# simonsobs/Pixell.jl

Measured on AMD Instinct MI355X. Metric: Mpix/s CAR bilinear reproject (Float64) + % HBM roofline, 1/2/4/8 MI355X, higher is better.
Workload: dtype f64

## Files before the change

### pixell.jl_amd/csrc/pxl_kernels.hip

```cpp
#include <hip/hip_runtime.h>

#include <algorithm>
#include <mutex>
#include <vector>
#include <cmath>
#include <cstdarg>
#include <cstdio>
#include <cstring>
#include <new>
#include <type_traits>

#include "pxl_device.h"

using namespace pxl;

static thread_local char g_err[512] = "";

static int fail(int code, const char* fmt, ...) {
    va_list ap;
    va_start(ap, fmt);
    vsnprintf(g_err, sizeof(g_err), fmt, ap);
    va_end(ap);
    return code;
}
#define HIP_TRY(expr)                                                                         \
    do {                                                                                      \
        hipError_t e_ = (expr);                                                               \
        if (e_ != hipSuccess) return fail(PXL_EHIP, "%s: %s", #expr, hipGetErrorString(e_));  \
    } while (0)

static int check_launch(const char* what) {
    hipError_t e = hipGetLastError();
    if (e != hipSuccess) return fail(PXL_EHIP, "launch of %s failed: %s", what, hipGetErrorString(e));
    return PXL_OK;
}

static bool wcs_ok(const pxl_car_wcs* w) {
    if (!w) return false;
    for (int k = 0; k < 2; ++k)
        if (!std::isfinite(w->cdelt[k]) || !std::isfinite(w->crpix[k]) || !std::isfinite(w->crval[k]) ||
            w->cdelt[k] == 0.0)
            return false;
    return std::isfinite(w->unit) && w->unit != 0.0;
}

static inline unsigned stream_grid(int64_t work_items, int block) {
    int64_t nb = (work_items + block - 1) / block;
    if (nb < 1) nb = 1;
    if (nb > (1LL << 20)) nb = 1LL << 20;
    return (unsigned)nb;
}

static int env_int(const char* name, int dflt) {
    const char* v = getenv(name);
    return (v && *v) ? atoi(v) : dflt;
}

#include "pxl_elementwise.h"
#include "pxl_unwrap.h"
#include "pxl_maps.h"
#include "pxl_fastmath.h"
#include "pxl_tan.h"
#include "pxl_reproject.h"
#include "pxl_reproject_dma.h"
#include "pxl_sample.h"
#include "pxl_misc.h"
#include "pxl_rccl.h"
#include "pxl_spread.h"
#include "pxl_distance.h"
#include "pxl_spline.h"

static constexpr size_t PXL_RING_BYTES = 17 * 1024;
static constexpr int64_t PXL_MIN_TILES = 8192;

struct pxl_reproject_plan {
    pxl_car_wcs win, wout;
    int64_t nx, ny, nc, src_row0, src_nrows;
    int64_t nxo, nyo, dst_row0, dst_nrows;
    int periodic;
    int device;
    int32_t* xi0; double* xfx; int32_t* yj0; double* yfy;
    void* table_mem;
    int32_t* h_yj0;
    int variant;
    int pairs;
    int pairs_dma;
    int seg_dma;
    int pairs_dma32;
    int seg_dma32;
    bool dma32_ok;
    int dypos;
    int rh;
    int rh32;
    int seg;
    int dxpos;
    int ns, pf;
    int nt;
    double* zero_page;
    bool staged_ok;
    bool vec_load;
    bool tables_built;
    hipStream_t comm_stream;
    hipEvent_t ev_ready, ev_halo;
    int64_t cov_have_lo, cov_have_hi, cov_lo, cov_hi;
};

struct UnwindWs {
    char* base;
    int8_t* c; int32_t* rloc; int32_t* bsum; int32_t* boff;
    int32_t* flag;
    unsigned long long* firstnan;
    int2* wsum; double2* wprev;
    UwLink* links; unsigned int* ticket; int64_t nlinks;
    int64_t nb, nw;
    int U;
    bool multipass;
};

static const int64_t kUnwindBlockFallbackMax = 1LL << 22;


static std::mutex g_pool_mu;
static hipMemPool_t g_pools[64] = {};
static hipMemPool_t unwind_pool() {
    std::mutex& mu = g_pool_mu;
    hipMemPool_t* pools = g_pools;
    int dev = 0;
    if (hipGetDevice(&dev) != hipSuccess || dev < 0 || dev >= 64) return nullptr;
    std::lock_guard<std::mutex> lock(mu);
    if (!pools[dev]) {
        hipMemPoolProps props = {};
        props.allocType = hipMemAllocationTypePinned;
        props.location.type = hipMemLocationTypeDevice;
        props.location.id = dev;
        hipMemPool_t p = nullptr;
        if (hipMemPoolCreate(&p, &props) != hipSuccess) { (void)hipGetLastError(); return nullptr; }
        uint64_t keep = ~0ull;
        (void)hipMemPoolSetAttribute(p, hipMemPoolAttrReleaseThreshold, &keep);
        pools[dev] = p;
    }
    return pools[dev];
}

static int unwind_ws_alloc(int64_t n, int nrow, hipStream_t st, UnwindWs* w) {
    w->nb = (n + PXL_SCAN_BLOCK - 1) / PXL_SCAN_BLOCK;
    int64_t U = n / (64 * 4096);
    U = U < 4 ? 4 : (U > 32 ? 32 : U);
    U &= ~(int64_t)(PXL_UW_G - 1);
    w->U = (int)U;
    w->nw = (n + 64 * U - 1) / (64 * U);
    if (w->nb > 0x7fffffffLL || w->nw > 0x7fffffffLL || n > 0x7fffffffLL) return fail(PXL_EINVAL, "unwind: batch too long (2^31 points)");
    auto up = [](size_t b) { return (b + 255) & ~(size_t)255; };
    w->multipass = n > kUnwindBlockFallbackMax;
    const size_t bytes_c = w->multipass ? up((size_t)nrow * n) : 0, bytes_r = w->multipass ? up((size_t)4 * nrow * n) : 0,
                 bytes_b = w->multipass ? up((size_t)4 * nrow * w->nb) : 0;
    const size_t bytes_ws = up((size_t)w->nw * sizeof(int2)), bytes_wp = up((size_t)w->nw * sizeof(double2));
    w->nlinks = (n + PXL_UW1_CHUNK - 1) / PXL_UW1_CHUNK;
    const size_t bytes_ln = up((size_t)w->nlinks * sizeof(UwLink) + 16);
    const size_t total = bytes_c + bytes_r + 2 * bytes_b + bytes_ws + bytes_wp + bytes_ln + 256;
    w->base = nullptr;
    hipMemPool_t pool = unwind_pool();
    if (pool) HIP_TRY(hipMallocFromPoolAsync((void**)&w->base, total, pool, st));
    else HIP_TRY(hipMallocAsync((void**)&w->base, total, st));
    char* p = w->base;
    w->c = (int8_t*)p; p += bytes_c;
    w->rloc = (int32_t*)p; p += bytes_r;
    w->bsum = (int32_t*)p; p += bytes_b;
    w->boff = (int32_t*)p; p += bytes_b;
    w->wsum = (int2*)p; p += bytes_ws;
    w->wprev = (double2*)p; p += bytes_wp;
    w->links = (UwLink*)p; w->ticket = (unsigned int*)(p + (size_t)w->nlinks * sizeof(UwLink)); p += bytes_ln;
    w->flag = (int32_t*)p;
    w->firstnan = (unsigned long long*)(p + 16);
    if (hipMemsetAsync(w->flag, 0, 32, st) != hipSuccess) {
        (void)hipFreeAsync(w->base, st);
        return fail(PXL_EHIP, "unwind: hipMemsetAsync failed");
    }
    return PXL_OK;
}

static int unwind_ws_free(UnwindWs* w, hipStream_t st, int rc) {
    hipError_t e = hipFreeAsync(w->base, st);
    if (e != hipSuccess && rc == PXL_OK) rc = fail(PXL_EHIP, "unwind: hipFreeAsync: %s", hipGetErrorString(e));
    return rc;
}

template <class SRC>
static int unwind_fused(const SRC& src, typename SRC::raw_t* out, int64_t n, bool inplace, UnwindWs& w, hipStream_t st) {
    const dim3 grid((unsigned)w.nw), block(64);
    int32_t* fastflag = w.flag + 2;
    hipLaunchKernelGGL((k_unwind_sums<SRC>), grid, block, 0, st, src, n, w.U, w.wsum, w.wprev, w.firstnan);
    hipLaunchKernelGGL(k_scan_wsums, dim3(1), dim3(1024), 0, st, w.nw, w.wsum);
    if (inplace) {
        hipLaunchKernelGGL((k_unwind_apply<SRC, false>), grid, block, 0, st, src, out, n, w.U, (const int2*)w.wsum,
                           (const double2*)w.wprev, (const unsigned long long*)w.firstnan, fastflag, (const int32_t*)nullptr);
        hipLaunchKernelGGL((k_unwind_apply<SRC, true>), grid, block, 0, st, src, out, n, w.U, (const int2*)w.wsum,
                           (const double2*)w.wprev, (const unsigned long long*)w.firstnan, fastflag, (const int32_t*)fastflag);
    } else {
        hipLaunchKernelGGL((k_unwind_apply<SRC, true>), grid, block, 0, st, src, out, n, w.U, (const int2*)w.wsum,
                           (const double2*)w.wprev, (const unsigned long long*)w.firstnan, fastflag, (const int32_t*)nullptr);
    }
    return check_launch("k_unwind fused");
}

template <class SRC>
static int unwind_onepass(const SRC& src, typename SRC::raw_t* out, int64_t n, UnwindWs& w, hipStream_t st) {
    if (w.nlinks > 0x7fffffffLL) return fail(PXL_EINVAL, "unwind: batch too long");
    hipError_t e = hipMemsetAsync(w.links, 0, (size_t)w.nlinks * sizeof(UwLink) + 16, st);
    if (e != hipSuccess) return fail(PXL_EHIP, "unwind: hipMemsetAsync: %s", hipGetErrorString(e));
    const int64_t nwg = (n + PXL_UW1_CHUNK - 1) / PXL_UW1_CHUNK;
    hipLaunchKernelGGL((k_unwind_onepass<SRC, PXL_UW1_U, PXL_UW1_UL>), dim3((unsigned)nwg), dim3(64 * PXL_UW1_WAVES), 0, st, src, out, n, w.links, w.ticket, w.flag + 2);
    return check_launch("k_unwind_onepass");
}

static int unwind_multipass(int64_t n, int nrow, double* sky, double period, double ref, UnwindWs& w, const int32_t* gate,
                            hipStream_t st) {
    int rc = PXL_OK;
    const unsigned cap = gate ? 2048u : 0xffffffffu;
    const unsigned g = std::min(stream_grid(n, 256), cap);
    const int64_t nb = w.nb;
    hipLaunchKernelGGL(k_unwrap_incr, dim3(g), dim3(256), 0, st, n, nrow, (const double*)sky, period, w.c, gate);
    for (int pass = 0; pass < 2 && rc == PXL_OK; ++pass) {
        const int32_t* pg = pass == 0 ? gate : w.flag;
        hipLaunchKernelGGL((k_scan_local<int8_t>), dim3(std::min((unsigned)nb, cap), nrow), dim3(256), 0, st, n, (const int8_t*)w.c, w.rloc, w.bsum, nb, pg);
        hipLaunchKernelGGL(k_scan_bsums, dim3(nrow), dim3(1024), 0, st, nb, (const int32_t*)w.bsum, w.boff, pg);
        hipLaunchKernelGGL(k_unwrap_verify, dim3(g), dim3(256), 0, st, n, nrow, (const double*)sky, period, w.c,
                           (const int32_t*)w.rloc, (const int32_t*)w.boff, nb, w.flag + pass, pg);
        rc = check_launch("k_unwrap scan/verify");
    }
    if (rc == PXL_OK) {
        hipLaunchKernelGGL(k_unwrap_apply, dim3(g), dim3(256), 0, st, n, nrow, sky, period, ref, (const int32_t*)w.rloc,
                           (const int32_t*)w.boff, nb, (const int32_t*)w.flag, gate);
        hipLaunchKernelGGL(k_unwind_rows, dim3(nrow), dim3(64), 0, st, n, nrow, sky, period, ref, 1, (const int32_t*)w.flag);
        rc = check_launch("k_unwrap_apply");
    }
    return rc;
}


extern "C" {

int pxl_version(void) { return PXL_VERSION; }

size_t pxl_last_error(char* buf, size_t n) {
    size_t len = strlen(g_err);
    if (buf && n) {
        size_t m = len < n - 1 ? len : n - 1;
        memcpy(buf, g_err, m);
        buf[m] = 0;
    }
// ... 269 lines not shown
    auto up256 = [](size_t b) { return (b + 255) & ~(size_t)255; };
    const size_t npix = (size_t)nx * (size_t)ny;
    const size_t b_csa = up256((size_t)nx * 16), b_csd = up256((size_t)ny * 16), b_best = up256(npix * 4), b_chain = npix * 8;
    hipStream_t st = (hipStream_t)stream;
    char* ws = nullptr;
    hipMemPool_t pool = unwind_pool();
    if (pool) HIP_TRY(hipMallocFromPoolAsync((void**)&ws, b_csa + b_csd + b_best + b_chain, pool, st));
    else HIP_TRY(hipMallocAsync((void**)&ws, b_csa + b_csd + b_best + b_chain, st));
    double2* csa = (double2*)ws;
    double2* csd = (double2*)(ws + b_csa);
    int32_t* best = (int32_t*)(ws + b_csa + b_csd);
    long long* chain = (long long*)(ws + b_csa + b_csd + b_best);
    hipLaunchKernelGGL(k_sdt_tables, dim3(stream_grid(nx + ny, 256)), dim3(256), 0, st, c, nx, ny, csa, csd);
    const size_t lds = (size_t)((nx + 63) / 64) * 16;
    hipLaunchKernelGGL(k_sdt_rows, dim3((unsigned)ny), dim3(PXL_SDT_ROW_THREADS), lds, st, m, nx, (const double2*)csa, best);
    hipLaunchKernelGGL(k_sdt_columns, dim3((unsigned)((nx + 63) / 64)), dim3(64), 0, st, (const int32_t*)best, nx, ny, up ? 1 : 0,
                       (const double2*)csa, (const double2*)csd, chain, dist);
    int rc = check_launch("k_sdt_rows / k_sdt_columns");
    hipError_t fe = hipFreeAsync(ws, st);
    if (fe != hipSuccess && rc == PXL_OK) rc = fail(PXL_EHIP, "distance_transform: hipFreeAsync: %s", hipGetErrorString(fe));
    return rc;
}

int pxl_sky2pix_tan_f64(const pxl_car_wcs* wcs, int64_t n, const double* ra, const double* dec, double* ipix,
                        double* jpix, void* stream) {
    if (!wcs_ok(wcs)) return fail(PXL_EINVAL, "sky2pix_tan: invalid WCS");
    if (n < 0 || (n > 0 && (!ipix || !jpix || !ra || !dec))) return fail(PXL_EINVAL, "sky2pix_tan: null buffer or negative n");
    if (n == 0) return PXL_OK;
    const bool vec = ((((uintptr_t)ra | (uintptr_t)dec | (uintptr_t)ipix | (uintptr_t)jpix) & 15) == 0);
    const dim3 grid(stream_grid((n + 1) / 2, 256));
    if (vec) hipLaunchKernelGGL((k_tan_points<true, false>), grid, dim3(256), 0, (hipStream_t)stream, tan_setup(*wcs), n, ra, dec, ipix, jpix);
    else     hipLaunchKernelGGL((k_tan_points<false, false>), grid, dim3(256), 0, (hipStream_t)stream, tan_setup(*wcs), n, ra, dec, ipix, jpix);
    return check_launch("k_tan_points (sky2pix)");
}

int pxl_pix2sky_tan_f64(const pxl_car_wcs* wcs, int64_t n, const double* ipix, const double* jpix, double* ra,
                        double* dec, void* stream) {
    if (!wcs_ok(wcs)) return fail(PXL_EINVAL, "pix2sky_tan: invalid WCS");
    if (n < 0 || (n > 0 && (!ipix || !jpix || !ra || !dec))) return fail(PXL_EINVAL, "pix2sky_tan: null buffer or negative n");
    if (n == 0) return PXL_OK;
    const bool vec = ((((uintptr_t)ra | (uintptr_t)dec | (uintptr_t)ipix | (uintptr_t)jpix) & 15) == 0);
    const dim3 grid(stream_grid((n + 1) / 2, 256));
    if (vec) hipLaunchKernelGGL((k_tan_points<true, true>), grid, dim3(256), 0, (hipStream_t)stream, tan_setup(*wcs), n, ipix, jpix, ra, dec);
    else     hipLaunchKernelGGL((k_tan_points<false, true>), grid, dim3(256), 0, (hipStream_t)stream, tan_setup(*wcs), n, ipix, jpix, ra, dec);
    return check_launch("k_tan_points (pix2sky)");
}

int pxl_posmap_tan_f64(const pxl_car_wcs* wcs, const int64_t shape[2], int64_t row0, int64_t nrows, double* ra,
                       double* dec, void* stream) {
    if (!wcs_ok(wcs)) return fail(PXL_EINVAL, "posmap_tan: invalid WCS");
    int rc = check_rows("posmap_tan", shape, row0, nrows);
    if (rc) return rc;
    if (nrows == 0) return PXL_OK;
    if (!ra || !dec) return fail(PXL_EINVAL, "posmap_tan: null output");
    const int64_t nchunk = (shape[0] + 511) / 512;
    const int64_t nrb = (nrows + PXL_TAN_ROWS - 1) / PXL_TAN_ROWS;
    if (nchunk * nrb > 0x7fffffffLL) return fail(PXL_EINVAL, "posmap_tan: map too large for one launch");
    const bool vec = (shape[0] % 2 == 0) && ((((uintptr_t)ra | (uintptr_t)dec) & 15) == 0);
    const TanParams tp0 = tan_setup(*wcs);
    const bool grid_pays = fabs(tp0.uos) * PXL_TG_W <= 0.04 && fabs(tp0.cd0) >= 0.3;
    if (grid_pays && shape[0] >= PXL_TG_W && nrows >= 8) {
        const int64_t ntx = (shape[0] + PXL_TG_W - 1) / PXL_TG_W, nty = (nrows + PXL_TG_ROWS - 1) / PXL_TG_ROWS;
        int fronts = 8;
        if (nty < 4 * fronts) fronts = 1;
        const int64_t per = (nty + fronts - 1) / fronts, nbx = (ntx + 3) / 4;
        const int64_t nblk = per * fronts * nbx;
        if (nblk <= 0x7fffffffLL) {
            if (vec) hipLaunchKernelGGL((k_posmap_tan_grid<true>), dim3((unsigned)nblk), dim3(256), 0, (hipStream_t)stream, tp0, shape[0], row0, nrows, ntx, per, fronts, ra, dec);
            else     hipLaunchKernelGGL((k_posmap_tan_grid<false>), dim3((unsigned)nblk), dim3(256), 0, (hipStream_t)stream, tp0, shape[0], row0, nrows, ntx, per, fronts, ra, dec);
            return check_launch("k_posmap_tan_grid");
        }
    }
    const dim3 grid((unsigned)(nchunk * nrb));
    if (vec) hipLaunchKernelGGL((k_posmap_tan<true>), grid, dim3(256), 0, (hipStream_t)stream, tan_setup(*wcs), shape[0], row0, nrows, nchunk, ra, dec);
    else     hipLaunchKernelGGL((k_posmap_tan<false>), grid, dim3(256), 0, (hipStream_t)stream, tan_setup(*wcs), shape[0], row0, nrows, nchunk, ra, dec);
    return check_launch("k_posmap_tan");
}


int pxl_reproject_plan_create(const pxl_car_wcs* wcs_in, const int64_t shape_in[3], int64_t src_row0,
                              int64_t src_nrows, const pxl_car_wcs* wcs_out, const int64_t shape_out[2],
                              int64_t dst_row0, int64_t dst_nrows, pxl_reproject_plan** out) {
    if (!out) return fail(PXL_EINVAL, "plan_create: null plan pointer");
    *out = nullptr;
    if (!wcs_ok(wcs_in) || !wcs_ok(wcs_out)) return fail(PXL_EINVAL, "plan_create: invalid WCS");
    if (!shape_in || !shape_out) return fail(PXL_EINVAL, "plan_create: null shape");
    if (shape_in[0] < 1 || shape_in[1] < 1 || shape_in[2] < 1 || shape_out[0] < 1 || shape_out[1] < 1)
        return fail(PXL_EINVAL, "plan_create: shapes must be positive");
    if (shape_in[0] > 400000000 || shape_in[1] > 1000000000 || shape_out[0] > 1000000000 || shape_out[1] > 1000000000)
        return fail(PXL_EINVAL, "plan_create: axis too long (source RA axis <= 4e8, others <= 1e9 pixels)");
    if (src_row0 < 0 || src_nrows < 0 || src_row0 + src_nrows > shape_in[1])
        return fail(PXL_EINVAL, "plan_create: source window outside the map");
    if (dst_row0 < 0 || dst_nrows < 0 || dst_row0 + dst_nrows > shape_out[1])
        return fail(PXL_EINVAL, "plan_create: destination window outside the map");

    pxl_reproject_plan* pl = new (std::nothrow) pxl_reproject_plan();
    if (!pl) return fail(PXL_ENOMEM, "plan_create: host allocation failed");
    pl->cov_lo = 0; pl->cov_hi = -1;
    pl->win = *wcs_in; pl->wout = *wcs_out;
    pl->nx = shape_in[0]; pl->ny = shape_in[1]; pl->nc = shape_in[2];
    pl->src_row0 = src_row0; pl->src_nrows = src_nrows;
    pl->nxo = shape_out[0]; pl->nyo = shape_out[1];
    pl->dst_row0 = dst_row0; pl->dst_nrows = dst_nrows;
    pl->periodic = fabs((double)pl->nx * fabs(wcs_in->cdelt[0] * wcs_in->unit) - PXL_TWOPI_D) < 1e-8;
    pl->tables_built = false;

    hipError_t e = hipGetDevice(&pl->device);
    if (e != hipSuccess) { delete pl; return fail(PXL_ENODEV, "hipGetDevice: %s", hipGetErrorString(e)); }

    size_t nxo = (size_t)pl->nxo, nyo = (size_t)pl->nyo;
    size_t off_xfx = 0;
    size_t off_yfy = off_xfx + ((nxo * 8 + 15) & ~(size_t)15);
    size_t off_xi0 = off_yfy + ((nyo * 8 + 15) & ~(size_t)15);
    size_t off_yj0 = off_xi0 + ((nxo * 4 + 15) & ~(size_t)15);
    size_t off_zero = off_yj0 + ((nyo * 4 + 15) & ~(size_t)15);
    size_t total = off_zero + 64;
    e = hipMalloc(&pl->table_mem, total);
    if (e != hipSuccess) { delete pl; return fail(PXL_ENOMEM, "plan_create: hipMalloc(%zu): %s", total, hipGetErrorString(e)); }
    char* base = (char*)pl->table_mem;
    e = hipMemset(base + off_zero, 0, 64);
    if (e != hipSuccess) { (void)hipFree(pl->table_mem); delete pl; return fail(PXL_EHIP, "plan_create: hipMemset: %s", hipGetErrorString(e)); }
    pl->zero_page = (double*)(base + off_zero);
    pl->xfx = (double*)(base + off_xfx); pl->yfy = (double*)(base + off_yfy);
    pl->xi0 = (int32_t*)(base + off_xi0); pl->yj0 = (int32_t*)(base + off_yj0);

    pl->h_yj0 = new (std::nothrow) int32_t[nyo];
    if (!pl->h_yj0) { (void)hipFree(pl->table_mem); delete pl; return fail(PXL_ENOMEM, "plan_create: host allocation failed"); }
    CarAffine co = car_affine(pl->wout);
    Sky2Pix si = sky2pix_setup(pl->win, pl->nx, pl->ny, 1, PXL_FORM_DIV);
    for (int64_t j = 0; j < pl->nyo; ++j) {
        double fr;
        split_cell(s2p_y(si, p2s_dec(co, (double)(j + 1))), &pl->h_yj0[j], &fr);
    }

    double sx = fabs((pl->wout.cdelt[0] * pl->wout.unit) / (pl->win.cdelt[0] * pl->win.unit));
    pl->dxpos = ((pl->wout.cdelt[0] * pl->wout.unit) / (pl->win.cdelt[0] * pl->win.unit)) > 0 ? 1 : 0;
    pl->dypos = ((pl->wout.cdelt[1] * pl->wout.unit) / (pl->win.cdelt[1] * pl->win.unit)) > 0 ? 1 : 0;
    double sy = fabs((pl->wout.cdelt[1] * pl->wout.unit) / (pl->win.cdelt[1] * pl->win.unit));
    pl->rh = env_int("PXL_REPROJECT_RH", sy >= 1.5 ? 4 : (sy > 0.3 ? 16 : 8));
    if (pl->rh < 1) pl->rh = 1;
    if (pl->rh > 64) pl->rh = 64;
    pl->rh32 = env_int("PXL_REPROJECT_RH", 32);
    if (pl->rh32 < 1) pl->rh32 = 1;
    if (pl->rh32 > 64) pl->rh32 = 64;
    pl->ns = env_int("PXL_REPROJECT_NS", (double)pl->nx * (double)pl->ny * (double)pl->nc * 8.0 <= 128.0 * 1048576.0 ? 4 : 8);
    if (pl->ns < 4) pl->ns = 4;
    while (pl->ns & (pl->ns - 1)) pl->ns &= pl->ns - 1;
    if (pl->ns > 64) pl->ns = 64;
    {
        int want_pf = (int)ceil((pl->ns - 2) / (sy > 0.125 ? sy : 0.125));
        pl->pf = env_int("PXL_REPROJECT_PF", want_pf < 3 ? 3 : want_pf);
    }
    pl->nt = env_int("PXL_REPROJECT_NT", 1);
    if (pl->pf < 0) pl->pf = 0;
    const int max_seg = PXL_MAXCH * 128;
    auto seg_for = [&](int pairs) -> int64_t {
        double span = ceil((double)(128 * pairs) * sx) + 5.0;
        int64_t s = (int64_t)span;
        return (s + 1) & ~(int64_t)1;
    };
    int want = env_int("PXL_REPROJECT_PAIRS", sx <= 0.55 ? 4 : 2);
    if (want != 1 && want != 2 && want != 4) want = 2;
    pl->pairs_dma = want;
    while (pl->pairs_dma > 1 && seg_for(pl->pairs_dma) > max_seg) pl->pairs_dma >>= 1;
    pl->seg_dma = (int)std::min<int64_t>(seg_for(pl->pairs_dma), max_seg);
    pl->pairs = want > 2 ? 2 : want;
    if (seg_for(pl->pairs) > max_seg && pl->pairs == 2) pl->pairs = 1;
    int64_t seg = seg_for(pl->pairs);
    auto stageable = [&](int64_t sg) { return (sg <= max_seg) && !(pl->periodic && sg > pl->nx) && sy <= 3.0; };
    pl->staged_ok = stageable(seg) && stageable(seg_for(pl->pairs_dma));
    pl->seg = (int)(seg <= max_seg ? seg : max_seg);
    {
        const int max_seg32 = PXL_MAXCH * 256;
        auto seg_for32 = [&](int pairs) -> int64_t {
            double span = ceil((double)(256 * pairs) * sx) + 8.0;
            return ((int64_t)span + 3) & ~(int64_t)3;
        };
        pl->pairs_dma32 = env_int("PXL_REPROJECT_PAIRS", sx < 0.75 ? 1 : 2);
        if (pl->pairs_dma32 != 1 && pl->pairs_dma32 != 2 && pl->pairs_dma32 != 4) pl->pairs_dma32 = 2;
        while (pl->pairs_dma32 > 1 && seg_for32(pl->pairs_dma32) > max_seg32) pl->pairs_dma32 >>= 1;
        int64_t s32 = seg_for32(pl->pairs_dma32);
        pl->dma32_ok = (s32 <= max_seg32) && !(pl->periodic && s32 > pl->nx) && sy <= 3.0 && (pl->nx % 4 == 0);
        pl->seg_dma32 = (int)std::min<int64_t>(s32, max_seg32);
    }
    pl->vec_load = (pl->nx % 2 == 0);
    *out = pl;
    return PXL_OK;
}

int pxl_reproject_plan_set_variant(pxl_reproject_plan* pl, int variant) {
    if (!pl || variant < 0 || variant > 2) return fail(PXL_EINVAL, "set_variant: bad argument");
    pl->variant = variant;
    return PXL_OK;
}

int pxl_reproject_plan_destroy(pxl_reproject_plan* pl) {
    if (!pl) return PXL_OK;
    if (pl->comm_stream) {
        (void)hipStreamSynchronize(pl->comm_stream);
        (void)hipEventDestroy(pl->ev_ready);
        (void)hipEventDestroy(pl->ev_halo);
        (void)hipStreamDestroy(pl->comm_stream);
    }
    if (pl->table_mem) (void)hipFree(pl->table_mem);
    delete[] pl->h_yj0;
    delete pl;
    return PXL_OK;
}

int pxl_reproject_build_tables(pxl_reproject_plan* pl, void* stream) {
    if (!pl) return fail(PXL_EINVAL, "build_tables: null plan");
    CarAffine co = car_affine(pl->wout);
    Sky2Pix si = sky2pix_setup(pl->win, pl->nx, pl->ny, 1, PXL_FORM_DIV);
    hipLaunchKernelGGL(k_build_tables, dim3(stream_grid(pl->nxo + pl->nyo, 256)), dim3(256), 0,
                       (hipStream_t)stream, co, si, pl->nxo, pl->nyo, pl->xi0, pl->xfx, pl->yj0, pl->yfy);
    int rc = check_launch("k_build_tables");
    if (rc == PXL_OK) pl->tables_built = true;
    return rc;
}

static int reproject_rows_impl(pxl_reproject_plan* pl, const void* src, void* dst, int64_t r0, int64_t nr,
                               void* stream, int dtype) {
    if (!pl) return fail(PXL_EINVAL, "execute: null plan");
    if (r0 < 0 || nr < 0 || r0 + nr > pl->dst_nrows) return fail(PXL_EINVAL, "execute: rows outside the dst window");
    if (nr == 0) return PXL_OK;
    if (!dst || (!src && pl->src_nrows > 0)) return fail(PXL_EINVAL, "execute: null src/dst");
    if (!pl->tables_built) return fail(PXL_EINVAL, "execute_rows: tables not built");
    hipStream_t st = (hipStream_t)stream;
    const bool f32 = dtype == 4;

    ReprojParams p;
    memset(&p, 0, sizeof(p));
    p.src = src; p.dst = dst;
    p.xi0 = pl->xi0; p.xfx = pl->xfx; p.yj0 = pl->yj0; p.yfy = pl->yfy;
    p.nx = pl->nx; p.ny = pl->ny; p.src_row0 = pl->src_row0; p.src_nrows = pl->src_nrows;
    p.nxo = pl->nxo; p.dst_row0 = pl->dst_row0; p.dst_nrows = pl->dst_nrows;
    p.r0 = r0; p.nr = nr; p.nc = (int32_t)pl->nc; p.periodic = pl->periodic;

    const bool aligned = (((uintptr_t)src & 15) == 0);
    bool staged = f32 ? (pl->dma32_ok && aligned) : pl->staged_ok;
    if (pl->variant == 1) staged = false;
    if (!staged) {
        int64_t work = ((pl->nxo + 1) / 2) * nr;
        dim3 g(stream_grid(work, 256), (unsigned)pl->nc);
        if (f32) hipLaunchKernelGGL((k_reproject_gather<float>), g, dim3(256), 0, st, p);
        else     hipLaunchKernelGGL((k_reproject_gather<double>), g, dim3(256), 0, st, p);
        return check_launch("k_reproject_gather");
    }

    const bool vec = f32 ? true : (pl->vec_load && aligned);
    const bool use_dma = f32 ? true : (vec && pl->variant != 2);
    const int pairs = f32 ? pl->pairs_dma32 : (use_dma ? pl->pairs_dma : pl->pairs);
    const int cw = f32 ? 256 : 128;
    const int TW = cw * pairs;
    p.seg = f32 ? pl->seg_dma32 : (use_dma ? pl->seg_dma : pl->seg);
    p.dxpos = pl->dxpos; p.dypos = pl->dypos;
    p.ntx = (int32_t)((pl->nxo + TW - 1) / TW);
    int rh = f32 ? pl->rh32 : pl->rh;
    while (rh > 4 && (int64_t)p.ntx * ((nr + rh - 1) / rh) * pl->nc < PXL_MIN_TILES) rh >>= 1;
    p.rh = rh;
    p.nty = (int32_t)((nr + rh - 1) / rh);
    p.ntiles = (int64_t)p.ntx * p.nty * pl->nc;
    p.tiles_per_xcd = (p.ntiles + 7) / 8;
    const int64_t nblocks = 8 * p.tiles_per_xcd;
    if (nblocks > 0x7fffffffLL) return fail(PXL_EINVAL, "execute: too many tiles (%lld)", (long long)nblocks);
    dim3 grid((unsigned)nblocks), block(64);
    if (use_dma) {
        const size_t esz = f32 ? 4 : 8;
        p.ns = pl->ns; p.pf = pl->pf; p.zero_page = pl->zero_page;
        p.nt = pl->nt != 0;
        while ((size_t)p.ns * p.seg * esz > PXL_RING_BYTES && p.ns > 4) p.ns >>= 1;
        size_t dma_lds = (size_t)p.ns * (size_t)p.seg * esz;
        const int nch = (p.seg + cw - 1) / cw;
        if (f32) return launch_reproject_dma_t<float>(pairs, nch, grid, dma_lds, st, p);
        return launch_reproject_dma_t<double>(pairs, nch, grid, dma_lds, st, p);
    }
    size_t lds_bytes = (size_t)PXL_NS * (size_t)pl->seg * sizeof(double);
    if (pl->pairs == 2) {
        if (vec) hipLaunchKernelGGL((k_reproject_staged<2, true>), grid, block, lds_bytes, st, p);
        else     hipLaunchKernelGGL((k_reproject_staged<2, false>), grid, block, lds_bytes, st, p);
    } else {
        if (vec) hipLaunchKernelGGL((k_reproject_staged<1, true>), grid, block, lds_bytes, st, p);
        else     hipLaunchKernelGGL((k_reproject_staged<1, false>), grid, block, lds_bytes, st, p);
    }
    return check_launch("k_reproject_staged");
}

int pxl_reproject_execute_rows(pxl_reproject_plan* pl, const double* src, double* dst, int64_t r0, int64_t nr,
                               void* stream) {
    return reproject_rows_impl(pl, src, dst, r0, nr, stream, 8);
}

int pxl_reproject_execute_rows_f32(pxl_reproject_plan* pl, const float* src, float* dst, int64_t r0, int64_t nr,
                                   void* stream) {
    return reproject_rows_impl(pl, src, dst, r0, nr, stream, 4);
}

int pxl_reproject_execute(pxl_reproject_plan* pl, const double* src, double* dst, void* stream) {
    int rc = pxl_reproject_build_tables(pl, stream);
    if (rc) return rc;
    return pxl_reproject_execute_rows(pl, src, dst, 0, pl->dst_nrows, stream);
}

int pxl_reproject_execute_f32(pxl_reproject_plan* pl, const float* src, float* dst, void* stream) {
    int rc = pxl_reproject_build_tables(pl, stream);
    if (rc) return rc;
    return pxl_reproject_execute_rows_f32(pl, src, dst, 0, pl->dst_nrows, stream);
}

int pxl_reproject_plan_src_rows(const pxl_reproject_plan* pl, int64_t* lo, int64_t* hi) {
    if (!pl || !lo || !hi) return fail(PXL_EINVAL, "plan_src_rows: null argument");
    int64_t l = INT64_MAX, h = INT64_MIN;
    for (int64_t r = 0; r < pl->dst_nrows; ++r) {
        int64_t j0 = pl->h_yj0[pl->dst_row0 + r];
        for (int64_t j = j0; j <= j0 + 1; ++j)
            if (j >= 1 && j <= pl->ny) { if (j - 1 < l) l = j - 1; if (j > h) h = j; }
    }
    if (l > h) { l = 0; h = 0; }
    *lo = l; *hi = h;
    return PXL_OK;
}

int pxl_reproject_plan_rows_covered(const pxl_reproject_plan* pl, int64_t have_lo, int64_t have_hi, int64_t* lo,
                                    int64_t* hi) {
    if (!pl || !lo || !hi) return fail(PXL_EINVAL, "plan_rows_covered: null argument");
    int64_t best_lo = 0, best_hi = 0, cur_lo = -1;
    for (int64_t r = 0; r <= pl->dst_nrows; ++r) {
        bool ok = false;
        if (r < pl->dst_nrows) {
            int64_t j0 = pl->h_yj0[pl->dst_row0 + r];
            ok = true;
            for (int64_t j = j0; j <= j0 + 1; ++j)
                if (j >= 1 && j <= pl->ny && !(j - 1 >= have_lo && j - 1 < have_hi)) ok = false;
        }
        if (ok) { if (cur_lo < 0) cur_lo = r; }
        else if (cur_lo >= 0) {
            if (r - cur_lo > best_hi - best_lo) { best_lo = cur_lo; best_hi = r; }
            cur_lo = -1;
        }
    }
    *lo = best_lo; *hi = best_hi;
    return PXL_OK;
}

static int sharded_step_impl(pxl_reproject_plan* pl, void* src, void* dst, int64_t own_row0, int64_t own_nrows,
                             const pxl_halo_xfer* sends, int nsends, const pxl_halo_xfer* recvs, int nrecvs,
                             void* comm, void* stream, int dtype) {
    if (!pl || !src || !dst) return fail(PXL_EINVAL, "sharded_step: null plan or buffer");
    if (nsends < 0 || nrecvs < 0 || (nsends > 0 && !sends) || (nrecvs > 0 && !recvs)) return fail(PXL_EINVAL, "sharded_step: bad transfer lists");
    const int64_t lo = pl->src_row0, hi = pl->src_row0 + pl->src_nrows;
    if (own_row0 < lo || own_nrows < 0 || own_row0 + own_nrows > hi) return fail(PXL_EINVAL, "sharded_step: owned rows outside the plan's source window");
    hipStream_t st = (hipStream_t)stream;
    int rc = PXL_OK;
    const bool exchange = nsends + nrecvs > 0;
    if (exchange) {
        if (!comm) return fail(PXL_EINVAL, "sharded_step: transfers listed but no RCCL communicator");
        const RcclApi& nc = rccl_api(false);
        if (!nc.ok) return fail(PXL_ENODEV, "sharded_step: RCCL entry points not available: %s", nc.where);
        if (nc.own && !rccl_own_comm_has(comm))
            return fail(PXL_ENODEV, "sharded_step: the communicator was not created by pxl_comm_init_rank, and the only RCCL instance "
                                    "this library can see is one it loaded itself (%s): a foreign communicator belongs to another instance", nc.where);
        int nranks = 0, me = -1;
        if (nc.CommCount((ncclComm_t)comm, &nranks) != ncclSuccess || nc.CommUserRank((ncclComm_t)comm, &me) != ncclSuccess)
            return fail(PXL_EINVAL, "sharded_step: not a usable RCCL communicator");
        for (int pass = 0; pass < 2; ++pass) {
            const pxl_halo_xfer* x = pass == 0 ? sends : recvs;
            for (int i = 0; i < (pass == 0 ? nsends : nrecvs); ++i) {
                if (x[i].peer < 0 || x[i].peer >= nranks) return fail(PXL_EINVAL, "sharded_step: peer %d outside the communicator (%d ranks)", x[i].peer, nranks);
                if (x[i].nrows < 1 || x[i].row0 < lo || x[i].row0 + x[i].nrows > hi) return fail(PXL_EINVAL, "sharded_step: transfer rows outside the plan's source window");
                if (pass == 0 && (x[i].row0 < own_row0 || x[i].row0 + x[i].nrows > own_row0 + own_nrows))
                    return fail(PXL_EINVAL, "sharded_step: a rank can only send rows it owns");
            }
        }
        if (!pl->comm_stream) {
            HIP_TRY(hipStreamCreateWithFlags(&pl->comm_stream, hipStreamNonBlocking));
            HIP_TRY(hipEventCreateWithFlags(&pl->ev_ready, hipEventDisableTiming));
            HIP_TRY(hipEventCreateWithFlags(&pl->ev_halo, hipEventDisableTiming));
        }
        HIP_TRY(hipEventRecord(pl->ev_ready, st));
        HIP_TRY(hipStreamWaitEvent(pl->comm_stream, pl->ev_ready, 0));
        const size_t esz = (size_t)dtype;
        const ncclDataType_t dt = dtype == 4 ? ncclFloat32 : ncclFloat64;
        ncclResult_t r = nc.GroupStart();
        for (int i = 0; i < nsends && r == ncclSuccess; ++i)
            for (int64_t c = 0; c < pl->nc && r == ncclSuccess; ++c)
                r = nc.Send((const char*)src + ((c * pl->src_nrows + (sends[i].row0 - lo)) * pl->nx) * esz,
                            (size_t)(sends[i].nrows * pl->nx), dt, sends[i].peer, (ncclComm_t)comm, pl->comm_stream);
        for (int i = 0; i < nrecvs && r == ncclSuccess; ++i)
            for (int64_t c = 0; c < pl->nc && r == ncclSuccess; ++c)
                r = nc.Recv((char*)src + ((c * pl->src_nrows + (recvs[i].row0 - lo)) * pl->nx) * esz,
                            (size_t)(recvs[i].nrows * pl->nx), dt, recvs[i].peer, (ncclComm_t)comm, pl->comm_stream);
        const ncclResult_t rend = nc.GroupEnd();
        if (r == ncclSuccess) r = rend;
        if (r != ncclSuccess) return fail(PXL_EHIP, "sharded_step: RCCL send/recv failed: %s", nc.GetErrorString(r));
        HIP_TRY(hipEventRecord(pl->ev_halo, pl->comm_stream));
    }
    rc = pxl_reproject_build_tables(pl, stream);
    if (rc) return rc;
    int64_t i_lo = 0, i_hi = pl->dst_nrows;
    if (exchange) {
        if (pl->cov_have_lo != own_row0 || pl->cov_have_hi != own_row0 + own_nrows || pl->cov_hi < pl->cov_lo) {
            rc = pxl_reproject_plan_rows_covered(pl, own_row0, own_row0 + own_nrows, &pl->cov_lo, &pl->cov_hi);
            if (rc) return rc;
            pl->cov_have_lo = own_row0; pl->cov_have_hi = own_row0 + own_nrows;
        }
        i_lo = pl->cov_lo; i_hi = pl->cov_hi;
    }
    if (i_hi > i_lo) {
        rc = reproject_rows_impl(pl, src, dst, i_lo, i_hi - i_lo, stream, dtype);
        if (rc) return rc;
    }
    if (exchange) {
        HIP_TRY(hipStreamWaitEvent(st, pl->ev_halo, 0));
        if (i_hi > i_lo) {
            if (i_lo > 0) { rc = reproject_rows_impl(pl, src, dst, 0, i_lo, stream, dtype); if (rc) return rc; }
            if (i_hi < pl->dst_nrows) rc = reproject_rows_impl(pl, src, dst, i_hi, pl->dst_nrows - i_hi, stream, dtype);
        } else {
            rc = reproject_rows_impl(pl, src, dst, 0, pl->dst_nrows, stream, dtype);
        }
    }
    return rc;
}

// ... 476 lines not shown
```

### pixell.jl_amd/csrc/pxl_reproject.h

```cpp
#pragma once

__global__ __launch_bounds__(256) void k_build_tables(CarAffine out, Sky2Pix in, int64_t nxo, int64_t nyo,
                                                      int32_t* __restrict__ xi0, double* __restrict__ xfx,
                                                      int32_t* __restrict__ yj0, double* __restrict__ yfy) {
    int64_t stride = (int64_t)gridDim.x * blockDim.x;
    for (int64_t k = (int64_t)blockIdx.x * blockDim.x + threadIdx.x; k < nxo + nyo; k += stride) {
        if (k < nxo) {
            double a = p2s_ra(out, (double)(k + 1));
            split_cell(s2p_x(in, a), &xi0[k], &xfx[k]);
        } else {
            int64_t j = k - nxo;
            double d = p2s_dec(out, (double)(j + 1));
            split_cell(s2p_y(in, d), &yj0[j], &yfy[j]);
        }
    }
}

struct ReprojParams {
    const void* src;
    void* dst;
    const int32_t* xi0; const double* xfx;
    const int32_t* yj0; const double* yfy;
    int64_t nx, ny, src_row0, src_nrows;
    int64_t nxo, dst_row0, dst_nrows;
    int64_t r0, nr;
    int32_t nc, periodic;
    int32_t rh;
    int32_t seg;
    int32_t dxpos;
    int32_t dypos;
    int32_t ntx, nty;
    int64_t ntiles, tiles_per_xcd;
    int32_t ns, pf;
    int32_t nt;
    const double* zero_page;
};

__device__ inline int64_t xcd_tile(int64_t b, int64_t tiles_per_xcd) {
    return (b & 7) * tiles_per_xcd + (b >> 3);
}

template <typename T>
__global__ __launch_bounds__(256) void k_reproject_gather(ReprojParams p) {
    const int64_t npair = (p.nxo + 1) / 2;
    const int64_t total = npair * p.nr;
    const int c = blockIdx.y;
    SrcViewT<T> m{(const T*)p.src + (int64_t)c * p.nx * p.src_nrows, p.nx, p.ny, p.src_row0, p.src_nrows, p.periodic};
    T* dplane = (T*)p.dst + (int64_t)c * p.nxo * p.dst_nrows;
    int64_t stride = (int64_t)gridDim.x * blockDim.x;
    for (int64_t t = (int64_t)blockIdx.x * blockDim.x + threadIdx.x; t < total; t += stride) {
        int64_t rr = t / npair;
        int64_t i = (t - rr * npair) * 2;
        int64_t r = p.r0 + rr;
        int64_t j0 = p.yj0[p.dst_row0 + r];
        double fy = p.yfy[p.dst_row0 + r];
        int64_t o = r * p.nxo + i;
        dplane[o] = (T)bilerp_cells(m, p.xi0[i], p.xfx[i], j0, fy);
        if (i + 1 < p.nxo) dplane[o + 1] = (T)bilerp_cells(m, p.xi0[i + 1], p.xfx[i + 1], j0, fy);
    }
}

#define PXL_NS 4
#define PXL_MAXCH 5

template <bool VEC>
__device__ inline void load_row_regs(const ReprojParams& p, const double* plane, int64_t j, int64_t cbase0,
                                     int lane, double2 (&regs)[PXL_MAXCH]) {
    int64_t jr = j - 1 - p.src_row0;
    const bool row_ok = (j >= 1) && (j <= p.ny) && (jr >= 0) && (jr < p.src_nrows);
    const double* rowp = plane + (row_ok ? jr : 0) * p.nx;
#pragma unroll
    for (int ch = 0; ch < PXL_MAXCH; ++ch) {
        int k = ch * 128 + 2 * lane;
        double2 v = make_double2(0.0, 0.0);
        if (k < p.seg && row_ok) {
            int64_t u = cbase0 + k;
            if (VEC) {
                bool ok = true;
                if (p.periodic) { u %= p.nx; if (u < 0) u += p.nx; }
                else ok = (u >= 0) && (u < p.nx);
                if (ok) v = *reinterpret_cast<const double2*>(rowp + u);
            } else {
                int64_t u0 = u, u1 = u + 1;
                bool ok0 = true, ok1 = true;
                if (p.periodic) {
                    u0 %= p.nx; if (u0 < 0) u0 += p.nx;
                    u1 %= p.nx; if (u1 < 0) u1 += p.nx;
                } else {
                    ok0 = (u0 >= 0) && (u0 < p.nx);
                    ok1 = (u1 >= 0) && (u1 < p.nx);
                }
                if (ok0) v.x = rowp[u0];
                if (ok1) v.y = rowp[u1];
            }
        }
        regs[ch] = v;
    }
}

__device__ inline void store_row_lds(const ReprojParams& p, double* slot, int lane, const double2 (&regs)[PXL_MAXCH]) {
#pragma unroll
    for (int ch = 0; ch < PXL_MAXCH; ++ch) {
        int k = ch * 128 + 2 * lane;
        if (k < p.seg) *reinterpret_cast<double2*>(slot + k) = regs[ch];
    }
}

template <int PAIRS, bool VEC>
__global__ __launch_bounds__(64) void k_reproject_staged(ReprojParams p) {
    extern __shared__ __attribute__((aligned(16))) double lds[];
    const int lane = threadIdx.x;
    constexpr int TW = 128 * PAIRS;

    const int64_t t = xcd_tile(blockIdx.x, p.tiles_per_xcd);
    if (t >= p.ntiles) return;
    const int tx = (int)(t % p.ntx);
    const int64_t trest = t / p.ntx;
    const int ty = (int)(trest % p.nty);
    const int c = (int)(trest / p.nty);

    const double* splane = (const double*)p.src + (int64_t)c * p.nx * p.src_nrows;
    double* dplane = (double*)p.dst + (int64_t)c * p.nxo * p.dst_nrows;

    const int64_t c0 = (int64_t)tx * TW;
    const int64_t clast = (c0 + TW < p.nxo ? c0 + TW : p.nxo) - 1;
    const int64_t rb = p.r0 + (int64_t)ty * p.rh;
    const int64_t re = (rb + p.rh < p.r0 + p.nr) ? rb + p.rh : p.r0 + p.nr;

    const int64_t a = p.dxpos ? p.xi0[c0] : p.xi0[clast];
    const int64_t ua = a - 1;
    const int64_t cbase0 = ua & ~(int64_t)1;
    int dloc[PAIRS][2];
    double fx[PAIRS][2];
    bool act[PAIRS][2];
    bool fits = true;
#pragma unroll
    for (int q = 0; q < PAIRS; ++q) {
#pragma unroll
        for (int e = 0; e < 2; ++e) {
            int64_t col = c0 + q * 128 + 2 * lane + e;
            act[q][e] = col < p.nxo;
            int64_t i0 = act[q][e] ? p.xi0[col] : a;
            fx[q][e] = act[q][e] ? p.xfx[col] : 0.0;
            int64_t d = i0 - a;
            if (p.periodic) { d %= p.nx; if (d < 0) d += p.nx; }
            d += ua - cbase0;
            if (d < 0 || d + 1 >= p.seg) fits = false;
            dloc[q][e] = (int)d;
        }
    }
    const bool vec_store = ((p.nxo & 1) == 0) && (((uintptr_t)p.dst & 15) == 0);

    if (!__all(fits)) {
        SrcView m{splane, p.nx, p.ny, p.src_row0, p.src_nrows, p.periodic};
        for (int64_t r = rb; r < re; ++r) {
            int64_t j0 = p.yj0[p.dst_row0 + r];
            double fy = p.yfy[p.dst_row0 + r];
#pragma unroll
            for (int q = 0; q < PAIRS; ++q)
#pragma unroll
                for (int e = 0; e < 2; ++e) {
                    int64_t col = c0 + q * 128 + 2 * lane + e;
                    if (act[q][e]) dplane[r * p.nxo + col] = bilerp_cells(m, p.xi0[col], fx[q][e], j0, fy);
                }
        }
        return;
    }

    int64_t tag0 = INT64_MIN, tag1 = INT64_MIN, tag2 = INT64_MIN, tag3 = INT64_MIN;
    auto resident = [&](int64_t j) -> bool {
        int s = (int)(j & 3);
        int64_t tg = (s == 0) ? tag0 : (s == 1) ? tag1 : (s == 2) ? tag2 : tag3;
        return tg == j;
    };
    auto settag = [&](int64_t j) {
        int s = (int)(j & 3);
        if (s == 0) tag0 = j; else if (s == 1) tag1 = j; else if (s == 2) tag2 = j; else tag3 = j;
    };

    int my_j0 = 0;
    double my_fy = 0.0;
    if (rb + lane < re) { my_j0 = p.yj0[p.dst_row0 + rb + lane]; my_fy = p.yfy[p.dst_row0 + rb + lane]; }
    auto row_j0 = [&](int64_t r) -> int64_t { return (int64_t)__builtin_amdgcn_readlane(my_j0, (int)(r - rb)); };
    auto row_fy = [&](int64_t r) -> double {
        int lo = __builtin_amdgcn_readlane(__double2loint(my_fy), (int)(r - rb));
        int hi = __builtin_amdgcn_readlane(__double2hiint(my_fy), (int)(r - rb));
        return __hiloint2double(hi, lo);
// ... 56 lines not shown
```

### pixell.jl_amd/csrc/pxl_reproject_dma.h

```cpp
#pragma once

template <int N>
__device__ __forceinline__ void wait_vm() {
    asm volatile("s_waitcnt vmcnt(%0)" ::"n"(N) : "memory");
}

__device__ __forceinline__ void wait_vm_upto(int k) {
    if (k < 8) {
        if (k < 4) {
            if (k < 2) { if (k < 1) wait_vm<0>(); else wait_vm<1>(); }
            else       { if (k < 3) wait_vm<2>(); else wait_vm<3>(); }
        } else {
            if (k < 6) { if (k < 5) wait_vm<4>(); else wait_vm<5>(); }
            else       { if (k < 7) wait_vm<6>(); else wait_vm<7>(); }
        }
    } else if (k < 16) {
        if (k < 12) {
            if (k < 10) { if (k < 9) wait_vm<8>(); else wait_vm<9>(); }
            else        { if (k < 11) wait_vm<10>(); else wait_vm<11>(); }
        } else {
            if (k < 14) { if (k < 13) wait_vm<12>(); else wait_vm<13>(); }
            else        { if (k < 15) wait_vm<14>(); else wait_vm<15>(); }
        }
    } else {
        if (k < 24) { if (k < 20) wait_vm<16>(); else wait_vm<20>(); }
        else        { if (k < 32) wait_vm<24>(); else wait_vm<32>(); }
    }
}

__device__ __forceinline__ void glds16_saddr(const void* sbase, uint32_t voff, uint32_t lds_byte_addr) {
    asm volatile("s_mov_b32 m0, %2\n\ts_nop 4\n\tglobal_load_lds_dwordx4 %1, %0"
                 :: "s"(sbase), "v"(voff), "s"(lds_byte_addr) : "memory");
}
__device__ __forceinline__ void glds16_vaddr(const void* gsrc, uint32_t lds_byte_addr) {
    asm volatile("s_mov_b32 m0, %1\n\ts_nop 0\n\tglobal_load_lds_dwordx4 %0, off"
                 :: "v"(gsrc), "s"(lds_byte_addr) : "memory");
}

template <typename T, int PAIRS, int NCH>
__global__ __launch_bounds__(64) void k_reproject_dma(ReprojParams p) {
    extern __shared__ __attribute__((aligned(16))) unsigned char lds_raw[];
    T* const lds = reinterpret_cast<T*>(lds_raw);
    const int lane = threadIdx.x;
    constexpr int EPL = 16 / (int)sizeof(T);
    constexpr int CW = 64 * EPL;
    constexpr int TW = CW * PAIRS;

    const int64_t t = xcd_tile(blockIdx.x, p.tiles_per_xcd);
    if (t >= p.ntiles) return;
    const int tx = (int)(t % p.ntx);
    const int64_t trest = t / p.ntx;
    const int ty = (int)(trest % p.nty);
    const int c = (int)(trest / p.nty);

    const T* splane = (const T*)p.src + (int64_t)c * p.nx * p.src_nrows;
    T* dplane = (T*)p.dst + (int64_t)c * p.nxo * p.dst_nrows;

    const int64_t c0 = (int64_t)tx * TW;
    const int64_t clast = (c0 + TW < p.nxo ? c0 + TW : p.nxo) - 1;
    const int64_t rb = p.r0 + (int64_t)ty * p.rh;
    const int64_t re = (rb + p.rh < p.r0 + p.nr) ? rb + p.rh : p.r0 + p.nr;
    const int nrows = (int)(re - rb);

    const int64_t a = p.dxpos ? p.xi0[c0] : p.xi0[clast];
    const int64_t ua = a - 1;
    const int64_t cbase0 = ua - (((ua % EPL) + EPL) % EPL);
    int dloc[PAIRS][EPL];
    double fx[PAIRS][EPL];
    bool act[PAIRS][EPL];
    bool fits = true;
#pragma unroll
    for (int q = 0; q < PAIRS; ++q) {
#pragma unroll
        for (int e = 0; e < EPL; ++e) {
            int64_t col = c0 + q * CW + EPL * lane + e;
            act[q][e] = col < p.nxo;
            int64_t i0 = act[q][e] ? p.xi0[col] : a;
            fx[q][e] = act[q][e] ? p.xfx[col] : 0.0;
            int64_t d = i0 - a;
            if (p.periodic) { d %= p.nx; if (d < 0) d += p.nx; }
            d += ua - cbase0;
            if (d < 0 || d + 1 >= p.seg) fits = false;
            dloc[q][e] = (int)d;
        }
    }

    int my_j0 = 0;
    double my_fy = 0.0;
    if (lane < nrows) { my_j0 = p.yj0[p.dst_row0 + rb + lane]; my_fy = p.yfy[p.dst_row0 + rb + lane]; }
    const int dir = p.dypos ? 1 : -1;
    const int my_t0 = p.dypos ? my_j0 : -(my_j0 + 1);
    const double my_wa = p.dypos ? 1 - my_fy : my_fy;
    const double my_wb = p.dypos ? my_fy : 1 - my_fy;
    {
        int nxt = __shfl_down(my_t0, 1, 64);
        bool mono = (lane + 1 >= nrows) || (nxt >= my_t0);
        if (!mono) fits = false;
    }

    if (!__all(fits)) {
        SrcViewT<T> m{splane, p.nx, p.ny, p.src_row0, p.src_nrows, p.periodic};
        for (int64_t r = rb; r < re; ++r) {
            int64_t j0 = p.yj0[p.dst_row0 + r];
            double fy = p.yfy[p.dst_row0 + r];
#pragma unroll
            for (int q = 0; q < PAIRS; ++q)
#pragma unroll
                for (int e = 0; e < EPL; ++e) {
                    int64_t col = c0 + q * CW + EPL * lane + e;
                    if (act[q][e]) dplane[r * p.nxo + col] = (T)bilerp_cells(m, p.xi0[col], fx[q][e], j0, fy);
                }
        }
        return;
    }

    uint32_t voff[NCH];
#pragma unroll
    for (int ch = 0; ch < NCH; ++ch) {
        int64_t u = cbase0 + ch * CW + EPL * lane;
        bool ok = true;
        if (p.periodic) { u %= p.nx; if (u < 0) u += p.nx; }
        else ok = (u >= 0) && (u < p.nx);
        voff[ch] = ok ? (uint32_t)(u * (int64_t)sizeof(T)) : 0xFFFFFFFFu;
    }

    const uint32_t lds_base = (uint32_t)(uintptr_t)lds;
    const uint32_t slot_bytes = (uint32_t)p.seg * (uint32_t)sizeof(T);
    const int ns_mask = p.ns - 1;

    int tv_lo = 1, tv_hi = 0;
    {
        const int64_t jlo = (p.src_row0 + 1 > 1) ? p.src_row0 + 1 : 1;
        const int64_t jhi = (p.src_row0 + p.src_nrows < p.ny) ? p.src_row0 + p.src_nrows : p.ny;
        if (jhi >= jlo) {
            if (p.dypos) { tv_lo = (int)jlo; tv_hi = (int)jhi; } else { tv_lo = -(int)jhi; tv_hi = -(int)jlo; }
        }
    }
    const int64_t row_step = (int64_t)dir * p.nx * (int64_t)sizeof(T);
    int treq = __builtin_amdgcn_readlane(my_t0, 0) - 1;
    const char* next_row = (const char*)splane + ((int64_t)dir * (treq + 1) - 1 - p.src_row0) * p.nx * (int64_t)sizeof(T);
    const bool tail_full = (p.seg == NCH * CW);
    const bool in_tail = ((NCH - 1) * CW + EPL * lane) < p.seg;
    const uint32_t zero_off = 0u;

    int vm_total = 0;
    int marks = 0;
    auto issue_next = [&]() {
        ++treq;
        const bool valid = (treq >= tv_lo) && (treq <= tv_hi);
        const uint32_t slot_addr = lds_base + (uint32_t)(treq & ns_mask) * slot_bytes;
        if (p.periodic) {
            const void* base = valid ? (const void*)next_row : (const void*)p.zero_page;
#pragma unroll
            for (int ch = 0; ch < NCH; ++ch) {
                const uint32_t off = valid ? voff[ch] : zero_off;
                if (ch < NCH - 1 || tail_full) glds16_saddr(base, off, slot_addr + ch * 1024u);
                else if (in_tail) glds16_saddr(base, off, slot_addr + ch * 1024u);
            }
        } else {
#pragma unroll
            for (int ch = 0; ch < NCH; ++ch) {
                const void* g = (valid && voff[ch] != 0xFFFFFFFFu) ? (const void*)(next_row + voff[ch])
                                                                   : (const void*)p.zero_page;
                if (ch < NCH - 1 || tail_full) glds16_vaddr(g, slot_addr + ch * 1024u);
                else if (in_tail) glds16_vaddr(g, slot_addr + ch * 1024u);
            }
        }
        next_row += row_step;
        vm_total += NCH;
        marks = (lane == (treq & ns_mask)) ? vm_total : marks;
    };

    const bool vec_store = ((p.nxo % EPL) == 0) && (((uintptr_t)p.dst & 15) == 0);
    T* orow = dplane + rb * p.nxo + c0 + EPL * lane;

    double hA[PAIRS][EPL], hB[PAIRS][EPL], wx[PAIRS][EPL];
#pragma unroll
    for (int q = 0; q < PAIRS; ++q)
#pragma unroll
        for (int e = 0; e < EPL; ++e) { wx[q][e] = 1 - fx[q][e]; hA[q][e] = 0.0; hB[q][e] = 0.0; }
    auto hrow = [&](int tr, double (&h)[PAIRS][EPL]) {
        const T* R = lds + (tr & ns_mask) * p.seg;
#pragma unroll
        for (int q = 0; q < PAIRS; ++q)
#pragma unroll
            for (int e = 0; e < EPL; ++e) {
                const int d = dloc[q][e];
                h[q][e] = wx[q][e] * (double)R[d] + fx[q][e] * (double)R[d + 1];
            }
    };
    auto row_loop = [&](auto fast_tag, auto nt_tag) {
    constexpr bool FAST = decltype(fast_tag)::value;
    constexpr bool NT = decltype(nt_tag)::value;
    int th = INT32_MIN / 2;
    for (int rr = 0; rr < nrows; ++rr) {
        const int t0 = __builtin_amdgcn_readlane(my_t0, rr);
        {
            const int ra = (rr + p.pf < nrows) ? rr + p.pf : nrows - 1;
            int tmax = __builtin_amdgcn_readlane(my_t0, ra) + 1;
            const int tlim = t0 + p.ns - 1;
            if (tmax > tlim) tmax = tlim;
            while (treq < tmax) issue_next();
        }
        if (t0 != th) {
            wait_vm_upto(vm_total - __builtin_amdgcn_readlane(marks, (t0 + 1) & ns_mask));
            if (t0 == th + 1) {
#pragma unroll
                for (int q = 0; q < PAIRS; ++q)
#pragma unroll
                    for (int e = 0; e < EPL; ++e) hA[q][e] = hB[q][e];
            } else {
                hrow(t0, hA);
            }
            hrow(t0 + 1, hB);
            th = t0;
            asm volatile("s_waitcnt lgkmcnt(0)" ::: "memory");
        }
        const double wa = __hiloint2double(__builtin_amdgcn_readlane(__double2hiint(my_wa), rr),
                                           __builtin_amdgcn_readlane(__double2loint(my_wa), rr));
        const double wb = __hiloint2double(__builtin_amdgcn_readlane(__double2hiint(my_wb), rr),
                                           __builtin_amdgcn_readlane(__double2loint(my_wb), rr));
#pragma unroll
        for (int q = 0; q < PAIRS; ++q) {
            alignas(16) T v[EPL];
#pragma unroll
            for (int e = 0; e < EPL; ++e) v[e] = (T)(wa * hA[q][e] + wb * hB[q][e]);
            T* o = orow + q * CW;
            if (FAST) {
                typedef unsigned int u4v __attribute__((ext_vector_type(4)));
                if (NT) __builtin_nontemporal_store(*reinterpret_cast<const u4v*>(v), reinterpret_cast<u4v*>(o));
                else *reinterpret_cast<uint4*>(o) = *reinterpret_cast<const uint4*>(v);
            }
            else if (vec_store) { if (act[q][0]) *reinterpret_cast<uint4*>(o) = *reinterpret_cast<const uint4*>(v); }
            else {
#pragma unroll
                for (int e = 0; e < EPL; ++e) if (act[q][e]) o[e] = v[e];
            }
        }
        if (FAST) vm_total += PAIRS;
        orow += p.nxo;
    }
    };
    if (vec_store && (c0 + TW <= p.nxo)) {
        if (p.nt) row_loop(std::true_type{}, std::true_type{});
        else row_loop(std::true_type{}, std::false_type{});
    } else row_loop(std::false_type{}, std::false_type{});
}

template <typename T>
static int launch_reproject_dma_t(int pairs, int nch, dim3 grid, size_t lds_bytes, hipStream_t st, const ReprojParams& p) {
#define PXL_DMA_CASE(P, N) \
    if (pairs == P && nch == N) { hipLaunchKernelGGL((k_reproject_dma<T, P, N>), grid, dim3(64), lds_bytes, st, p); return check_launch("k_reproject_dma"); }
    PXL_DMA_CASE(1, 1) PXL_DMA_CASE(1, 2) PXL_DMA_CASE(1, 3) PXL_DMA_CASE(1, 4) PXL_DMA_CASE(1, 5)
    PXL_DMA_CASE(2, 1) PXL_DMA_CASE(2, 2) PXL_DMA_CASE(2, 3) PXL_DMA_CASE(2, 4) PXL_DMA_CASE(2, 5)
    PXL_DMA_CASE(4, 1) PXL_DMA_CASE(4, 2) PXL_DMA_CASE(4, 3) PXL_DMA_CASE(4, 4) PXL_DMA_CASE(4, 5)
#undef PXL_DMA_CASE
    return fail(PXL_EINVAL, "reproject: no LDS-DMA kernel for pairs=%d nch=%d", pairs, nch);
}
```

Measured before the change: 387,100.

## Trim tail-chunk DMA loads to used span and add optional non-temporal row loads

The tail chunk of each staged source row is now loaded only up to the largest column any lane actually reads (a wave-wide max of dloc), not the full segment width, which cuts redundant global-to-LDS traffic. Separately, an env-controlled option (off by default) issues global_load_lds with the nt hint, either for all rows or only for the tile's interior rows, so they bypass cache retention. Computing the per-tile span costs a shuffle reduction, and splitting the issue path into two instantiations grows code size.

```diff
diff --git a/pixell.jl_amd/csrc/pxl_kernels.hip b/pixell.jl_amd/csrc/pxl_kernels.hip
--- a/pixell.jl_amd/csrc/pxl_kernels.hip
+++ b/pixell.jl_amd/csrc/pxl_kernels.hip
@@ -96,6 +96,7 @@
     int dxpos;
     int ns, pf;
     int nt;
+    int ntload;
     double* zero_page;
     bool staged_ok;
     bool vec_load;
@@ -671,6 +672,8 @@
         pl->pf = env_int("PXL_REPROJECT_PF", want_pf < 3 ? 3 : want_pf);
     }
     pl->nt = env_int("PXL_REPROJECT_NT", 1);
+    pl->ntload = env_int("PXL_REPROJECT_NTLOAD", 0);
+    if (pl->ntload < 0 || pl->ntload > 2) pl->ntload = 0;
     if (pl->pf < 0) pl->pf = 0;
     const int max_seg = PXL_MAXCH * 128;
     auto seg_for = [&](int pairs) -> int64_t {
@@ -788,6 +791,7 @@
         const size_t esz = f32 ? 4 : 8;
         p.ns = pl->ns; p.pf = pl->pf; p.zero_page = pl->zero_page;
         p.nt = pl->nt != 0;
+        p.ntload = pl->ntload;
         while ((size_t)p.ns * p.seg * esz > PXL_RING_BYTES && p.ns > 4) p.ns >>= 1;
         size_t dma_lds = (size_t)p.ns * (size_t)p.seg * esz;
         const int nch = (p.seg + cw - 1) / cw;
diff --git a/pixell.jl_amd/csrc/pxl_reproject.h b/pixell.jl_amd/csrc/pxl_reproject.h
--- a/pixell.jl_amd/csrc/pxl_reproject.h
+++ b/pixell.jl_amd/csrc/pxl_reproject.h
@@ -33,6 +33,7 @@
     int64_t ntiles, tiles_per_xcd;
     int32_t ns, pf;
     int32_t nt;
+    int32_t ntload;
     const double* zero_page;
 };
 
diff --git a/pixell.jl_amd/csrc/pxl_reproject_dma.h b/pixell.jl_amd/csrc/pxl_reproject_dma.h
--- a/pixell.jl_amd/csrc/pxl_reproject_dma.h
+++ b/pixell.jl_amd/csrc/pxl_reproject_dma.h
@@ -28,13 +28,23 @@
     }
 }
 
+template <bool NTL>
 __device__ __forceinline__ void glds16_saddr(const void* sbase, uint32_t voff, uint32_t lds_byte_addr) {
-    asm volatile("s_mov_b32 m0, %2\n\ts_nop 4\n\tglobal_load_lds_dwordx4 %1, %0"
-                 :: "s"(sbase), "v"(voff), "s"(lds_byte_addr) : "memory");
-}
+    if (NTL)
+        asm volatile("s_mov_b32 m0, %2\n\ts_nop 4\n\tglobal_load_lds_dwordx4 %1, %0 nt"
+                     :: "s"(sbase), "v"(voff), "s"(lds_byte_addr) : "memory");
+    else
+        asm volatile("s_mov_b32 m0, %2\n\ts_nop 4\n\tglobal_load_lds_dwordx4 %1, %0"
+                     :: "s"(sbase), "v"(voff), "s"(lds_byte_addr) : "memory");
+}
+template <bool NTL>
 __device__ __forceinline__ void glds16_vaddr(const void* gsrc, uint32_t lds_byte_addr) {
-    asm volatile("s_mov_b32 m0, %1\n\ts_nop 0\n\tglobal_load_lds_dwordx4 %0, off"
-                 :: "v"(gsrc), "s"(lds_byte_addr) : "memory");
+    if (NTL)
+        asm volatile("s_mov_b32 m0, %1\n\ts_nop 0\n\tglobal_load_lds_dwordx4 %0, off nt"
+                     :: "v"(gsrc), "s"(lds_byte_addr) : "memory");
+    else
+        asm volatile("s_mov_b32 m0, %1\n\ts_nop 0\n\tglobal_load_lds_dwordx4 %0, off"
+                     :: "v"(gsrc), "s"(lds_byte_addr) : "memory");
 }
 
 template <typename T, int PAIRS, int NCH>
@@ -139,33 +149,52 @@
     const int64_t row_step = (int64_t)dir * p.nx * (int64_t)sizeof(T);
     int treq = __builtin_amdgcn_readlane(my_t0, 0) - 1;
     const char* next_row = (const char*)splane + ((int64_t)dir * (treq + 1) - 1 - p.src_row0) * p.nx * (int64_t)sizeof(T);
-    const bool tail_full = (p.seg == NCH * CW);
-    const bool in_tail = ((NCH - 1) * CW + EPL * lane) < p.seg;
+    int dmax = 0;
+#pragma unroll
+    for (int q = 0; q < PAIRS; ++q)
+#pragma unroll
+        for (int e = 0; e < EPL; ++e) dmax = dloc[q][e] + 1 > dmax ? dloc[q][e] + 1 : dmax;
+#pragma unroll
+    for (int m = 32; m >= 1; m >>= 1) { const int o = __shfl_xor(dmax, m, 64); dmax = o > dmax ? o : dmax; }
+    const bool in_tail = (lane == 0) || (((NCH - 1) * CW + EPL * lane) <= dmax);
+    const bool tail_full = __all(in_tail);
     const uint32_t zero_off = 0u;
+    int nt_lo = 0, nt_hi = 0;
+    if (p.ntload == 1) { nt_lo = INT32_MIN; nt_hi = INT32_MAX; }
+    else if (p.ntload == 2) {
+        const int t_first = __builtin_amdgcn_readlane(my_t0, 0), t_last = __builtin_amdgcn_readlane(my_t0, nrows - 1) + 1;
+        nt_lo = t_first > tv_lo - 1 ? t_first : tv_lo - 1;
+        nt_hi = t_last < tv_hi + 1 ? t_last : tv_hi + 1;
+    }
 
     int vm_total = 0;
     int marks = 0;
+    auto issue_row = [&](auto ntl_tag, bool valid, uint32_t slot_addr) {
+        constexpr bool NTL = decltype(ntl_tag)::value;
+        if (p.periodic) {
+            const void* base = valid ? (const void*)next_row : (const void*)p.zero_page;
+#pragma unroll
+            for (int ch = 0; ch < NCH; ++ch) {
+                const uint32_t off = valid ? voff[ch] : zero_off;
+                if (ch < NCH - 1 || tail_full) glds16_saddr<NTL>(base, off, slot_addr + ch * 1024u);
+                else if (in_tail) glds16_saddr<NTL>(base, off, slot_addr + ch * 1024u);
+            }
+        } else {
+#pragma unroll
+            for (int ch = 0; ch < NCH; ++ch) {
+                const void* g = (valid && voff[ch] != 0xFFFFFFFFu) ? (const void*)(next_row + voff[ch])
+                                                                   : (const void*)p.zero_page;
+                if (ch < NCH - 1 || tail_full) glds16_vaddr<NTL>(g, slot_addr + ch * 1024u);
+                else if (in_tail) glds16_vaddr<NTL>(g, slot_addr + ch * 1024u);
+            }
+        }
+    };
     auto issue_next = [&]() {
         ++treq;
         const bool valid = (treq >= tv_lo) && (treq <= tv_hi);
         const uint32_t slot_addr = lds_base + (uint32_t)(treq & ns_mask) * slot_bytes;
-        if (p.periodic) {
-            const void* base = valid ? (const void*)next_row : (const void*)p.zero_page;
-#pragma unroll
-            for (int ch = 0; ch < NCH; ++ch) {
-                const uint32_t off = valid ? voff[ch] : zero_off;
-                if (ch < NCH - 1 || tail_full) glds16_saddr(base, off, slot_addr + ch * 1024u);
-                else if (in_tail) glds16_saddr(base, off, slot_addr + ch * 1024u);
-            }
-        } else {
-#pragma unroll
-            for (int ch = 0; ch < NCH; ++ch) {
-                const void* g = (valid && voff[ch] != 0xFFFFFFFFu) ? (const void*)(next_row + voff[ch])
-                                                                   : (const void*)p.zero_page;
-                if (ch < NCH - 1 || tail_full) glds16_vaddr(g, slot_addr + ch * 1024u);
-                else if (in_tail) glds16_vaddr(g, slot_addr + ch * 1024u);
-            }
-        }
+        if (treq > nt_lo && treq < nt_hi) issue_row(std::true_type{}, valid, slot_addr);
+        else issue_row(std::false_type{}, valid, slot_addr);
         next_row += row_step;
         vm_total += NCH;
         marks = (lane == (treq & ns_mask)) ? vm_total : marks;
```

New measurement: 387,200 (median of 6 runs). Within noise of the previous version (+0.0%).
